# jwheo12/RustRayTrace

Measured on AMD Instinct MI355X. Metric: Mrays/sec + wall-clock for 1920×1080×512spp RTOW final scene, higher is better.
Workload: dtype f32; 1 GPU; C2 RTOW final scene (gpu/mod.rs generator, seed 0x5EED1234), 1920x1080x512spp, max_depth 100, 486 spheres; spp=512, max_depth=100, parallelism=whole frame on 1 GPU (the band split with one rank), no gather

## Files before the change

include/rrt_hip.h:

```cpp
#ifndef RRT_HIP_H
#define RRT_HIP_H

#include <stddef.h>
#include <stdint.h>

#ifdef __cplusplus
extern "C" {
#endif

#define RRT_ABI_VERSION 11u


typedef struct RrtCamera {
    float origin[4];
    float pixel00[4];
    float pixel_delta_u[4];
    float pixel_delta_v[4];
    float u[4];
    float v[4];
    float background[4];
    float params_f[4];
    uint32_t params_u[4];
} RrtCamera;

// ... 301 lines not shown
int32_t rrt_quantize_accum_books_async(uint32_t n_pixels, const float *d_accum, uint32_t samples_per_pixel,
                                       uint8_t *d_rgb8, void *stream);
int32_t rrt_quantize_accum_books_f64_async(uint32_t n_pixels, const double *d_accum, uint32_t samples_per_pixel,
                                           uint8_t *d_rgb8, void *stream);

int32_t rrt_hip_render_f64_rgb8(const RrtCamera *cam,
                                const RrtSphere *spheres, uint32_t n_spheres,
                                const RrtMaterial *materials, uint32_t n_materials,
                                const RrtTexture *textures, uint32_t n_textures,
                                uint32_t total_spp, uint32_t n_gpus, uint32_t flags,
                                uint8_t *rgb8_out);

int32_t rrt_format_pnm_from_rgb8(uint32_t width, uint32_t height, const uint8_t *rgb8, int32_t binary,
                                 char *buf, size_t cap, size_t *written);
int32_t rrt_write_pnm_from_rgb8(uint32_t width, uint32_t height, const uint8_t *rgb8, int32_t binary,
                                const char *path);

int32_t rrt_device_count(int32_t *count);

void rrt_testing_device_wrap(int32_t on);

void rrt_testing_f64_layout(int32_t layout);

typedef struct RrtLaunchPlanQuery {
    uint32_t n_nodes, n_prims, stack_depth, node_stride;
    uint32_t book, specular, image_tex, n_perlin;
    uint32_t n_media, n_quads, f64, bvh4_in_lds;
    uint32_t min_waves, global_waves, _pad[2];
} RrtLaunchPlanQuery;
typedef struct RrtLaunchPlan {
    uint32_t ok, f64;
    int32_t kernel_class, shape;
    uint32_t stack_bytes, threads, waves, waves_noise_free;
    uint32_t scene_in_lds, perlin_in_lds, inv_r_in_lds, rec32_in_lds;
    uint32_t raise_limit, _pad;
    uint64_t lds_bytes;
} RrtLaunchPlan;
int32_t rrt_testing_launch_plan(const RrtLaunchPlanQuery *query, RrtLaunchPlan *plan);

int32_t rrt_testing_recip_check(uint64_t *mismatches);

int32_t rrt_testing_trig32_check(double *out);

int32_t rrt_testing_sqrt64_check(uint64_t *out);

enum RrtDeviceOp {
// ... 37 lines not shown
```

rustraytrace_amd/_lib.py:

```python
from __future__ import annotations

import ctypes
import os
from ctypes import POINTER, c_char_p, c_double, c_float, c_int32, c_size_t, c_uint8, c_uint32, c_uint64, c_void_p

import numpy as np

PKG_DIR = os.path.dirname(os.path.abspath(__file__))
LIB_PATH = os.environ.get("RRT_LIB_PATH") or os.path.join(PKG_DIR, "librrt_hip.so")

CAMERA_DTYPE = np.dtype(
    [
        ("origin", "<f4", 4),
        ("pixel00", "<f4", 4),
        ("pixel_delta_u", "<f4", 4),
        ("pixel_delta_v", "<f4", 4),
        ("u", "<f4", 4),
        ("v", "<f4", 4),
        ("background", "<f4", 4),
        ("params_f", "<f4", 4),
        ("params_u", "<u4", 4),
    ]
)
SPHERE_DTYPE = np.dtype([("center_radius", "<f4", 4), ("material_index", "<u4"), ("_pad", "<u4", 3)])
# ... 31 lines not shown
    "rrt_hip_render_rgb8",
    "rrt_hip_render_rgb8_ex",
    "rrt_quantize_accum_books",
    "rrt_quantize_accum_async",
    "rrt_format_pnm_from_rgb8",
    "rrt_write_pnm_from_rgb8",
    "rrt_hip_render_ex",
    "rrt_scene_create_ex",
    "rrt_build_bvh_ex",
    "rrt_build_bvh_binned",
    "rrt_scene_read_bvh",
    "rrt_build_next_week_scene",
    "rrt_build_rest_of_your_life_scene",
    "rrt_flatten_scene",
    "rrt_device_count",
    "rrt_hip_render_f64",
    "rrt_render_tile_f64_async",
    "rrt_quantize_accum_books_f64",
    "rrt_quantize_accum_books_async",
    "rrt_quantize_accum_books_f64_async",
    "rrt_hip_render_f64_rgb8",
    "rrt_testing_device_wrap",
    "rrt_testing_f64_layout",
    "rrt_testing_launch_plan",
    "rrt_testing_recip_check",
    "rrt_testing_trig32_check",
    "rrt_testing_sqrt64_check",
    "rrt_testing_device_ops",
    "rrt_testing_div_check",
    "rrt_testing_device_ops64",
)

DEVICE_OPS = {
    "SIN": (0, 1, 1), "COS": (1, 1, 1), "LOG": (2, 1, 1), "ACOS": (3, 1, 1), "ATAN2": (4, 2, 1),
    "DIV_A": (5, 2, 4), "DIV_CONST": (6, 1, 4), "FLOOR_I32": (7, 1, 1), "CHECKER": (8, 4, 1),
    "PERLIN": (9, 3, 8), "VEC": (10, 9, 13), "QUAD": (11, 9, 2), "SPHERE": (12, 11, 13),
}

DEVICE_OPS64 = {
    "ACOS64": (0, 1, 1), "ATAN2_64": (1, 2, 1), "DIV_A64": (2, 2, 3), "DIV_CONST64": (3, 1, 4), "SQRT64": (4, 1, 1),
    "AS_I32": (5, 1, 1), "ATT64": (6, 2, 4), "VEC64": (7, 9, 11), "TEXEL64": (8, 5, 6), "SPHERE64": (9, 11, 6),
}


class RrtTexture(ctypes.Structure):
    _fields_ = [("rgb8", POINTER(c_uint8)), ("width", c_int32), ("height", c_int32)]
# ... 201 lines not shown
        "rrt_hip_render_rgb8_ex": (c_int32, [P, P, c_uint32, P, c_uint32, P, c_uint32, P, c_uint32, c_uint32, c_uint32,
                                             P]),
        "rrt_quantize_accum_async": (c_int32, [c_uint32, P, c_uint32, P, P]),
        "rrt_format_pnm_from_rgb8": (c_int32, [c_uint32, c_uint32, P, c_int32, P, c_size_t, P]),
        "rrt_write_pnm_from_rgb8": (c_int32, [c_uint32, c_uint32, P, c_int32, c_char_p]),
        "rrt_hip_render_ex": (c_int32, [P, P, c_uint32, P, c_uint32, P, c_uint32, P, c_uint32, c_uint32, c_uint32, P]),
        "rrt_scene_create_ex": (c_int32, [P, P, c_uint32, P, c_uint32, P, c_uint32, P, c_uint32, c_int32, P]),
        "rrt_build_bvh_ex": (c_int32, [P, c_uint32, P, c_uint32, c_uint32, P, c_size_t, P, P]),
        "rrt_build_bvh_binned": (c_int32, [P, c_uint32, P, c_uint32, c_double, c_uint32, P, c_size_t, P, P]),
        "rrt_scene_read_bvh": (c_int32, [P, P, c_size_t, P]),
        "rrt_build_next_week_scene": (c_int32, [c_int32, P, c_uint64, P]),
        "rrt_build_rest_of_your_life_scene": (c_int32, [P, c_uint64, P]),
        "rrt_flatten_scene": (c_int32, [P, c_uint32, P, c_uint32, c_uint32, P]),
        "rrt_device_count": (c_int32, [P]),
        "rrt_hip_render_f64": (c_int32, [P, P, c_uint32, P, c_uint32, P, c_uint32, c_uint32, c_uint32, c_uint32, P]),
        "rrt_render_tile_f64_async": (c_int32, [P, P, P, P]),
        "rrt_quantize_accum_books_f64": (c_int32, [c_uint32, c_uint32, P, c_uint32, P]),
        "rrt_quantize_accum_books_async": (c_int32, [c_uint32, P, c_uint32, P, P]),
        "rrt_quantize_accum_books_f64_async": (c_int32, [c_uint32, P, c_uint32, P, P]),
        "rrt_hip_render_f64_rgb8": (c_int32, [P, P, c_uint32, P, c_uint32, P, c_uint32, c_uint32, c_uint32, c_uint32,
                                              P]),
        "rrt_testing_device_wrap": (None, [c_int32]),
        "rrt_testing_f64_layout": (None, [c_int32]),
        "rrt_testing_launch_plan": (c_int32, [P, P]),
        "rrt_testing_recip_check": (c_int32, [P]),
        "rrt_testing_trig32_check": (c_int32, [P]),
        "rrt_testing_sqrt64_check": (c_int32, [P]),
        "rrt_testing_device_ops": (c_int32, [c_uint32, c_uint32, P, P, P]),
        "rrt_testing_device_ops64": (c_int32, [c_uint32, c_uint32, P, P, P]),
        "rrt_testing_div_check": (c_int32, [P, c_uint32, P]),
    }
    experiment = "RRT_LIB_PATH" in os.environ
    for name, (res, args) in sig.items():
        if experiment and not hasattr(lib, name):
            continue
        fn = getattr(lib, name)
        fn.restype = res
        fn.argtypes = args
    _LIB = lib
    return lib


def check(rc: int) -> None:
    if rc != 0:
        msg = load().rrt_hip_last_error()
        raise RrtError(rc, msg.decode() if msg else "")
# ... 27 lines not shown
```

rustraytrace_amd/csrc/rrt_books64.hip:

```cpp
#include "rrt_internal.h"
#include "../../include/rrt_hip.h"

#include <atomic>
#include <cstdlib>
#include <type_traits>

namespace rrt {
namespace {

#include "rrt_device.h"
#include "rrt_box32.h"
#include "rrt_sphere32.h"

constexpr int kPrioRefill = 2, kPrioNode = 1, kPrioLeaf = 2, kPrioShade = 0;

#ifndef RRT_F64_STATS
#define RRT_F64_STATS 0
#endif
#ifndef RRT_DEBUG_NOREJECT
#define RRT_DEBUG_NOREJECT 0
#endif
__device__ __forceinline__ uint32_t wave_max_u32(uint32_t v) {
#pragma unroll
    for (int off = 32; off > 0; off >>= 1) v = max(v, (uint32_t)__shfl_xor((int)v, off, 64));
// ... 393 lines not shown
    uint32_t rx, ry, rz;
};
__device__ __forceinline__ RayK64 ray_consts64(D3 o, D3 d) {
    RayK64 r;
    r.b = box32_ray(o.x, o.y, o.z, d.x, d.y, d.z);
    r.ox = r.b.ix < 0.0f ? 16u : 0u;
    r.oy = r.b.iy < 0.0f ? 48u : 32u;
    r.oz = r.b.iz < 0.0f ? 80u : 64u;
    r.rx = r.b.ix < 0.0f ? 16u : 0u;
    r.ry = r.b.iy < 0.0f ? 16u : 0u;
    r.rz = r.b.iz < 0.0f ? 16u : 0u;
    return r;
}

struct Trav64 {
    double closest;
    float closest32;
    int hit_prim;
    int node;
    int sp;
};

template <bool kCount, typename Node, typename Stack>
__device__ __forceinline__ bool trav_node64(const Node *__restrict__ nodes, Stack &stack, const RayK64 &rk,
                                            Trav64 &t, Leaves &lv, Counters &cnt) {
    if (kCount) { cnt.nodes++; cnt.boxes += 2; }
    bool h0, h1;
    uint32_t l0, l1;
    float tn0 = 0.0f, tn1 = 0.0f;
    if constexpr (std::is_same<Node, GNode>::value) {
        const char *bx = reinterpret_cast<const char *>(nodes) + __umul24((uint32_t)t.node, 112u);
        auto quad = [&](uint32_t byte_off) { return *reinterpret_cast<const float4 *>(bx + byte_off); };
        const float4 x = quad(rk.ox), y = quad(rk.oy), z = quad(rk.oz);
        h0 = box32_hit(x.x, x.y, y.x, y.y, z.x, z.y, rk.b, t.closest32, tn0);
        h1 = box32_hit(x.z, x.w, y.z, y.w, z.z, z.w, rk.b, t.closest32, tn1);
        const uint2 lk = *reinterpret_cast<const uint2 *>(bx + 96);
        l0 = lk.x;
        l1 = lk.y;
    } else {
        const uint4 *q = reinterpret_cast<const uint4 *>(nodes + t.node);
        const uint4 a = q[0], b = q[1];
        auto ord = [](uint32_t w, uint32_t r) { return __builtin_amdgcn_alignbit(w, w, r); };
        const uint32_t x0 = ord(a.x, rk.rx), y0 = ord(a.y, rk.ry), z0 = ord(a.z, rk.rz);
        const uint32_t x1 = ord(a.w, rk.rx), y1 = ord(b.x, rk.ry), z1 = ord(b.y, rk.rz);
        h0 = box32_hit(lo16(x0), hi16(x0), lo16(y0), hi16(y0), lo16(z0), hi16(z0), rk.b, t.closest32, tn0);
        h1 = box32_hit(lo16(x1), hi16(x1), lo16(y1), hi16(y1), lo16(z1), hi16(z1), rk.b, t.closest32, tn1);
        l0 = b.z;
        l1 = b.w;
    }
    const uint32_t c0 = h0 ? (l0 >> kLinkCountShift) : 0u;
    const uint32_t c1 = h1 ? (l1 >> kLinkCountShift) : 0u;
    lv = c0 ? l0 + (c1 << kLinkCountShift) : l1;
    if (c0) h0 = false;
    if (c1) h1 = false;
    if (h0 && h1) {
        const bool first1 = tn1 < tn0;
        stack.store(t.sp, first1 ? (int)l0 : (int)l1);
        ++t.sp;
        t.node = first1 ? (int)l1 : (int)l0;
    } else if (h0) {
        t.node = (int)l0;
    } else if (h1) {
        t.node = (int)l1;
    } else if (t.sp == 0) {
        t.node = -1;
    } else {
        --t.sp;
        t.node = stack.load(t.sp);
    }
    return (c0 | c1) != 0;
}

__device__ __forceinline__ double recip_a64(double a) {
    if (!(a >= 0x1.0p-64 && a <= 0x1.0p64)) return 0.0;
    double r = __builtin_amdgcn_rcp(a);
    double e = __builtin_fma(-a, r, 1.0);
    r = __builtin_fma(r, e, r);
    e = __builtin_fma(-a, r, 1.0);
    return __builtin_fma(r, e, r);
}
__device__ __forceinline__ double div_a64_short(double n, double a, double ra) {
    const double q = n * ra;
    return __builtin_fma(__builtin_fma(-a, q, n), ra, q);
}
__device__ __forceinline__ bool div_a64_in_band(double r) { return __builtin_fabs(r) >= 0x1.0p-896; }
__device__ __forceinline__ double div_a64(double n, double a, double ra) {
    const double r = div_a64_short(n, a, ra);
    return div_a64_in_band(r) ? r : n / a;
}
__device__ __forceinline__ double root64(double h, double sq, double a, double ra) {
    const double n1 = h - sq, n2 = h + sq;
    double root = div_a64_short(n1, a, ra);
    if (!(0.001 < root)) root = div_a64_short(n2, a, ra);
// ... 325 lines not shown
        const uint32_t min_active = (live * P.trav_frac) >> 8;
        const uint32_t leaf_min = (live * P.leaf_frac) >> 8;
        if constexpr (RRT_F64_STATS == 1) {
            const uint64_t t = __builtin_amdgcn_s_memtime();
            ph0 += t - tp;
            tp = t;
        }
        RayK64 rk;
        double a = 0.0;
        if (tr.node >= 0) {
            rk = ray_consts64(ps.o, ps.d);
            a = dot(ps.d, ps.d);
        }
        __builtin_amdgcn_s_setprio(kPrioNode);
        Leaves lv = 0;
        for (;;) {
            if constexpr (RRT_F64_STATS == 4) {
                const uint64_t sm = __ballot(tr.node >= 0 && lv == 0);
                if (sm != 0) {
                    ph0 += 1;
                    ph1 += (uint64_t)__popcll(sm);
                }
            }
            if (tr.node >= 0 && lv == 0) {
                Leaves l;
                if (trav_node64<kCount>(nodes, stack, rk, tr, l, cnt)) lv = l;
            }
            const uint64_t pm = __ballot(lv != 0);
            const uint64_t tm = __ballot(tr.node >= 0) | pm;
            const bool leave = (uint32_t)__popcll(tm) <= min_active;
            const bool batch = ((uint32_t)__popcll(pm) > leaf_min) | leave | (tm == pm);
            if ((pm != 0) & batch) {
                __builtin_amdgcn_s_setprio(kPrioLeaf);
                [[maybe_unused]] const uint32_t n_l = lv >> kLinkCountShift, s_l = cnt.d1;
                if (lv != 0) {
                    leaves64<kCount>(prims, recs32, lv, ps.o, ps.d, a, P.sphere32 != 0u, tr, cnt);
                    lv = 0;
                }
                if constexpr (RRT_F64_STATS == 2) {
                    ph0 += wave_max_u32(n_l);
                    ph1 += wave_max_u32(cnt.d1 - s_l);
                    ph2 += 1;
                }
                if constexpr (RRT_F64_STATS == 4) ph2 += 64;
                __builtin_amdgcn_s_setprio(kPrioNode);
            }
            if (leave) break;
        }
        if constexpr (RRT_F64_STATS == 1) {
            const uint64_t t = __builtin_amdgcn_s_memtime();
// ... 561 lines not shown
```

rustraytrace_amd/csrc/rrt_device.h:

```cpp
#pragma once

__device__ __forceinline__ uint32_t wave_slot() {
    return (uint32_t)__builtin_amdgcn_readfirstlane(threadIdx.x) == threadIdx.x ? 64u : 0u;
}

__device__ __forceinline__ float lo16(uint32_t v) { return (float)__builtin_bit_cast(_Float16, (uint16_t)(v & 0xffffu)); }
__device__ __forceinline__ float hi16(uint32_t v) { return (float)__builtin_bit_cast(_Float16, (uint16_t)(v >> 16)); }

__device__ __forceinline__ uint64_t splitmix64(uint64_t z) {
    z += 0x9e3779b97f4a7c15ull;
    z = (z ^ (z >> 30)) * 0xbf58476d1ce4e5b9ull;
    z = (z ^ (z >> 27)) * 0x94d049bb133111ebull;
    return z ^ (z >> 31);
}
struct RngState {
    uint32_t a, b, c, d;
};
__device__ __forceinline__ uint32_t rotl32(uint32_t x, int k) { return (x << k) | (x >> (32 - k)); }
__device__ __forceinline__ uint32_t xor3_32(uint32_t x, uint32_t y, uint32_t z) {
#if defined(__gfx950__)
    return __builtin_amdgcn_bitop3_b32(x, y, z, 0x96);
#else
    return x ^ y ^ z;
#endif
// ... 17 lines not shown
    s.c ^= s.a;
    s.d ^= s.b;
    s.b ^= s.c;
    s.a ^= s.d;
    s.c ^= t;
    s.d = rotl32(s.d, 11);
    return r;
}
__device__ __forceinline__ RngState rng_seed(uint64_t z, uint64_t key) {
    return RngState{(uint32_t)z, (uint32_t)(z >> 32), (uint32_t)key, (uint32_t)(key >> 32) | 1u};
}
__device__ __forceinline__ uint64_t rng_key(const RngState &s) { return (uint64_t)s.a | ((uint64_t)s.b << 32); }
__device__ __forceinline__ float rnd(RngState &s) { return (float)(rng_next(s) >> 8) * 0x1.0p-24f; }
__device__ __forceinline__ float rnd_range(RngState &s, float lo, float hi) { return rnd(s) * (hi - lo) + lo; }
__device__ __forceinline__ float rnd_pm1(RngState &s) {
    return __builtin_fmaf((float)(rng_next(s) >> 8), 0x1.0p-23f, -1.0f);
}

struct Counters {
    uint32_t nodes, boxes, spheres;
    uint32_t d0, d1, d2;
};

template <typename StackT, int kBlk>
struct LdsStack {
    StackT *base;
    __device__ __forceinline__ void init(StackT *lds, uint32_t tid) {
        if constexpr (sizeof(StackT) == 2) {
            const uint32_t lane = tid & 63u;
            base = lds + (tid & ~63u) + ((lane & 31u) << 1) + (lane >> 5);
        } else {
            base = lds + tid;
        }
    }
    __device__ __forceinline__ void store(int sp, int v) { base[sp * kBlk] = (StackT)v; }
    __device__ __forceinline__ int load(int sp) const { return (int)base[sp * kBlk]; }
};

using Leaves = uint32_t;

__device__ __forceinline__ const __attribute__((address_space(4))) KParams *kernarg_params() {
    auto q = (const __attribute__((address_space(4))) KParams *)__builtin_amdgcn_kernarg_segment_ptr();
    asm volatile("" : "+s"(q));
    return q;
}
template <class FD>
__device__ __forceinline__ FastDiv fdiv(const FD &f) { return FastDiv{f.m, f.s}; }

template <class KP>
__device__ __forceinline__ uint64_t pixel_key(const KP &P, uint32_t x, uint32_t y) {
    return splitmix64(((uint64_t)P.seed << 32) ^ (uint64_t)(y * P.width + x));
}
__device__ __forceinline__ RngState path_rng_k(uint64_t key, uint32_t s) { return rng_seed(splitmix64(key + s), key); }

template <class KP>
__host__ __device__ __forceinline__ uint32_t chunk_first(const KP &P, uint32_t c) {
    return c < P.n_big ? c * P.chunk : P.n_big * P.chunk + (c - P.n_big) * P.chunk_small;
}

// ... 6 lines not shown
```

rustraytrace_amd/csrc/rrt_host.cpp:

```cpp
#include "rrt_internal.h"
#include "rrt_bvh_binned.h"
#include "../../include/rrt_hip.h"

#include <algorithm>
#include <limits>
#include <atomic>
#include <chrono>
#include <cmath>
#include <cstdio>
#include <cstdlib>
#include <cstring>
#include <functional>
#include <mutex>
#include <string>
#include <thread>
#include <vector>

namespace {

thread_local std::string g_err;

int fail(int code, const std::string &msg) {
    g_err = msg;
    return code;
// ... 1838 lines not shown
    const size_t elem = scene->f64 ? sizeof(rrt::D4) : sizeof(float4);
    HIP_TRY(hipMalloc((void **)&scratch, std::max<size_t>((size_t)p.tile_rows * p.width, 1) * elem),
            "hipMalloc scratch accum");
    p.accum = scratch;
    p.accum64 = reinterpret_cast<rrt::D4 *>(scratch);
    p.counters = scene->d_work_counters;
    hipError_t e = hipMemset(scene->d_work_counters, 0, 8 * sizeof(unsigned long long));
    if (e == hipSuccess) e = rrt::launch_render_counting(p, nullptr);
    if (e == hipSuccess) e = hipDeviceSynchronize();
    unsigned long long c[8] = {0};
    if (e == hipSuccess) e = hipMemcpy(c, scene->d_work_counters, sizeof(c), hipMemcpyDeviceToHost);
    (void)hipFree(scratch);
    if (e != hipSuccess) return fail(RRT_E_HIP, std::string("counting render failed: ") + hipGetErrorString(e));
    *out = RrtCounters{c[0], c[1], c[2], c[3], c[4]};
    return RRT_OK;
}

}

static std::atomic<bool> g_device_wrap{false};
extern "C" void rrt_testing_device_wrap(int32_t on) { g_device_wrap.store(on != 0); }

extern "C" void rrt_testing_f64_layout(int32_t layout) { rrt::set_f64_layout(layout); }

extern "C" int32_t rrt_testing_launch_plan(const RrtLaunchPlanQuery *q, RrtLaunchPlan *out) {
    if (!q || !out) return fail(RRT_E_INVALID, "null query or out");
    *out = RrtLaunchPlan{};
    if (q->node_stride != 32u && q->node_stride != 80u && q->node_stride != 128u)
        return fail(RRT_E_INVALID, "node_stride must be 80 (staged BVH2), 32 (global BVH2) or 128 (BVH4)");
    if (q->book > 3u || q->book == 1u) return fail(RRT_E_INVALID, "book must be 0 (book 1), 2 or 3");
    rrt::KParams p{};
    static float4 some_motion;
    p.n_nodes = q->n_nodes;
    p.n_prims = q->n_prims;
    p.stack_depth = q->stack_depth;
    p.bvh_width = q->node_stride == 128u ? 4u : 2u;
    p.scene_in_lds = q->node_stride == 128u ? q->bvh4_in_lds : q->node_stride == 80u ? 1u : 0u;
    p.prim_motion = q->book ? &some_motion : nullptr;
    p.flags = (q->book == 3u ? RRT_FLAG_BOOK3 | RRT_FLAG_RAY_TIME : 0u) | (q->f64 ? RRT_FLAG_F64 : 0u);
    p.specular = q->specular;
    p.image_tex = q->image_tex;
    p.n_perlin = q->n_perlin;
    p.n_media = q->n_media;
    p.n_quads = q->n_quads;
    p.sphere32 = q->f64 ? 1u : 0u;
    p.min_waves = q->min_waves ? q->min_waves : 6u;
// ... 1200 lines not shown
```

rustraytrace_amd/csrc/rrt_internal.h:

```cpp
#pragma once

#include <hip/hip_runtime.h>
#include <stdint.h>

namespace rrt {

struct alignas(16) GNode {
    float box[2][9];
    uint32_t link[2];
};
static_assert(sizeof(GNode) == 80, "GNode must be 80 B");
struct alignas(16) GNodeH {
    uint32_t c0[3];
    uint32_t c1[3];
    uint32_t link[2];
};
static_assert(sizeof(GNodeH) == 32, "GNodeH must be 32 B");
constexpr uint32_t kLinkCountShift = 28;
constexpr uint32_t kLinkFirstMask = (1u << kLinkCountShift) - 1u;
constexpr uint32_t kMaxLeafPrims = 7;
constexpr uint32_t kMaxUnbounded = 4;

struct alignas(16) GNode4 {
    float4 lox, hix, loy, hiy, loz, hiz;
    int4 child;
    int4 count;
};
static_assert(sizeof(GNode4) == 128, "GNode4 must be 128 B");

struct alignas(16) GMaterial {
    float4 a;
    int4 b;
};

struct alignas(16) GPerlin {
    float4 randvec[256];
    uint32_t perm[256];
};

struct alignas(16) GQuad {
    float4 q;
    float4 u;
    float4 v;
// ... 246 lines not shown
```

rustraytrace_amd/csrc/rrt_kernel.hip:

```cpp
#include "rrt_internal.h"
#include "../../include/rrt_hip.h"

#include <algorithm>
#include <cstdio>
#include <cstdlib>
#include <type_traits>

namespace rrt {
namespace {

#ifndef RRT_PHASE_TIMING
#define RRT_PHASE_TIMING 0
#endif
#ifndef RRT_DEBUG_NOREJECT
#define RRT_DEBUG_NOREJECT 0
#endif
#ifndef RRT_DEBUG_EXTRA_NODE_LOAD
#define RRT_DEBUG_EXTRA_NODE_LOAD 0
#endif
#ifndef RRT_PRIO_REFILL
#define RRT_PRIO_REFILL 2
#endif
#ifndef RRT_PRIO_NODE
#define RRT_PRIO_NODE 1
#endif
#ifndef RRT_PRIO_LEAF
// ... 118 lines not shown
    if (x == 0.0f) {
        if (y > 0.0f) return kPiO2;
        if (y < 0.0f) return -kPiO2;
        return 0.0f;
    }
    float z = rrt_atanf(y / x);
    if (x < 0.0f) z = (y < 0.0f) ? z - kPi : z + kPi;
    return z;
}

__device__ __forceinline__ bool box_hit(float lx, float hx, float ly, float hy, float lz, float hz,
                                        V3 inv, V3 oi, float tmin, float tmax, float &tnear) {
    const float x0 = __builtin_fmaf(lx, inv.x, -oi.x), x1 = __builtin_fmaf(hx, inv.x, -oi.x);
    const float y0 = __builtin_fmaf(ly, inv.y, -oi.y), y1 = __builtin_fmaf(hy, inv.y, -oi.y);
    const float z0 = __builtin_fmaf(lz, inv.z, -oi.z), z1 = __builtin_fmaf(hz, inv.z, -oi.z);
    const float nr = __builtin_fmaxf(__builtin_fmaxf(__builtin_fminf(x0, x1), __builtin_fminf(y0, y1)),
                                     __builtin_fmaxf(__builtin_fminf(z0, z1), tmin));
    const float fr = __builtin_fminf(__builtin_fminf(__builtin_fmaxf(x0, x1), __builtin_fmaxf(y0, y1)),
                                     __builtin_fminf(__builtin_fmaxf(z0, z1), tmax));
    tnear = nr;
    return nr < fr;
}

__device__ __forceinline__ bool box_hit_ordered(float nx, float fx, float ny, float fy, float nz, float fz, V3 inv,
                                                V3 oi, float tmin, float tmax, float &tnear) {
    const float x0 = __builtin_fmaf(nx, inv.x, -oi.x), x1 = __builtin_fmaf(fx, inv.x, -oi.x);
    const float y0 = __builtin_fmaf(ny, inv.y, -oi.y), y1 = __builtin_fmaf(fy, inv.y, -oi.y);
    const float z0 = __builtin_fmaf(nz, inv.z, -oi.z), z1 = __builtin_fmaf(fz, inv.z, -oi.z);
    const float nr = __builtin_fmaxf(__builtin_fmaxf(x0, y0), __builtin_fmaxf(z0, tmin));
    const float fr = __builtin_fminf(__builtin_fminf(x1, y1), __builtin_fminf(z1, tmax));
    tnear = nr;
    return nr < fr;
}


struct RayK {
    V3 inv;
    V3 oi;
    float a;
    float ra;
    uint32_t ox, oy, oz;
};

__device__ __forceinline__ float clamp_inv(float v) { return __builtin_fmaxf(__builtin_fminf(v, 0x1.0p64f), -0x1.0p64f); }
__device__ __forceinline__ float clamped_slope(float s) {
    return __builtin_fabsf(s) < 0x1.0p-126f ? __builtin_copysignf(0x1.0p64f, s) : clamp_inv(recip_rn(s));
}

#ifndef RRT_F16_ORDERED_MAX_CLASS
#define RRT_F16_ORDERED_MAX_CLASS 3
#endif
#ifndef RRT_B1U_WAVES
#define RRT_B1U_WAVES 8
// ... 255 lines not shown
            cr = prim_cr.at(i);
        }
        const V3 oc = v3(cr.x - o.x, cr.y - o.y, cr.z - o.z);
        const float h = dot(d, oc);
        const float c = dot(oc, oc) - (PR::kR2 ? cr.w : cr.w * cr.w);
        const float disc = __builtin_fmaf(h, h, -(a * c));
        if (disc < 0.0f) continue;
        if constexpr (RRT_PHASE_TIMING == 3) cnt.d2 += 1;
        const float sq = sqrt_rn(disc);
        float root = div_by_a(h - sq, rk);
        if (!(0.001f < root)) root = div_by_a(h + sq, rk);
        if (0.001f < root && root < closest) {
            closest = root;
            hit_prim = i;
        }
    }
}


struct Trav {
    float closest;
    int hit_prim;
    int node;
    int sp;
};

__device__ __forceinline__ void trav_begin(Trav &t) {
    t.closest = __builtin_inff();
    t.hit_prim = -1;
    t.node = 0;
    t.sp = 0;
}


template <bool kCount, bool kOrd16, typename Node, typename Stack>
__device__ __forceinline__ bool trav_node(const Node *__restrict__ nodes, Stack &stack, const RayK &rk, Trav &t,
                                          Leaves &lv, Counters &cnt) {
    if (kCount) { cnt.nodes++; cnt.boxes += 2; }
    float tn0 = 0.0f, tn1 = 0.0f;
    bool h0, h1;
    uint32_t l0, l1;
    if constexpr (std::is_same<Node, GNode>::value) {
        const GNode &n = *reinterpret_cast<const GNode *>(reinterpret_cast<const char *>(nodes) +
                                                           __umul24((uint32_t)t.node, (uint32_t)sizeof(GNode)));
        const char *bx = reinterpret_cast<const char *>(&n.box[0][0]);
        auto plane = [&](uint32_t byte_off) { return *reinterpret_cast<const float *>(bx + byte_off); };
        h0 = box_hit_ordered(plane(rk.ox), plane(rk.ox + 4), plane(rk.oy), plane(rk.oy + 4), plane(rk.oz),
                             plane(rk.oz + 4), rk.inv, rk.oi, 0.001f, t.closest, tn0);
        h1 = box_hit_ordered(plane(rk.ox + 36), plane(rk.ox + 40), plane(rk.oy + 36), plane(rk.oy + 40),
                             plane(rk.oz + 36), plane(rk.oz + 40), rk.inv, rk.oi, 0.001f, t.closest, tn1);
        l0 = n.link[0];
        l1 = n.link[1];
    } else {
        const uint4 *q = reinterpret_cast<const uint4 *>(nodes + t.node);
        const uint4 a = q[0], b = q[1];
#if RRT_DEBUG_EXTRA_NODE_LOAD == 1
        {
            const uint4 *q2 = q;
            asm volatile("" : "+v"(q2));
            const uint4 c = q2[0];
            asm volatile("" ::"v"(c.x ^ c.y ^ c.z ^ c.w));
        }
#endif
#if RRT_DEBUG_EXTRA_NODE_LOAD == 2
        uint32_t dep_zero;
        {
            uint32_t z = a.x;
            asm volatile("v_and_b32 %0, 0, %0" : "+v"(z));
            const uint4 c = q[z];
            dep_zero = c.x;
            asm volatile("v_and_b32 %0, 0, %0" : "+v"(dep_zero));
        }
#endif
        if (kOrd16) {
            auto ord = [](uint32_t w, uint32_t r) { return __builtin_amdgcn_alignbit(w, w, r); };
            uint32_t ry, rz;
            asm volatile("v_lshrrev_b32 %0, 5, %1" : "=v"(ry) : "v"(rk.ox));
            asm volatile("v_lshrrev_b32 %0, 10, %1" : "=v"(rz) : "v"(rk.ox));
            const uint32_t x0 = ord(a.x, rk.ox), y0 = ord(a.y, ry), z0 = ord(a.z, rz);
            const uint32_t x1 = ord(a.w, rk.ox), y1 = ord(b.x, ry), z1 = ord(b.y, rz);
            h0 = box_hit_ordered(lo16(x0), hi16(x0), lo16(y0), hi16(y0), lo16(z0), hi16(z0), rk.inv, rk.oi, 0.001f,
                                 t.closest, tn0);
            h1 = box_hit_ordered(lo16(x1), hi16(x1), lo16(y1), hi16(y1), lo16(z1), hi16(z1), rk.inv, rk.oi, 0.001f,
                                 t.closest, tn1);
        } else {
            h0 = box_hit(lo16(a.x), hi16(a.x), lo16(a.y), hi16(a.y), lo16(a.z), hi16(a.z), rk.inv, rk.oi, 0.001f, t.closest, tn0);
            h1 = box_hit(lo16(a.w), hi16(a.w), lo16(b.x), hi16(b.x), lo16(b.y), hi16(b.y), rk.inv, rk.oi, 0.001f, t.closest, tn1);
        }
        l0 = b.z;
        l1 = b.w;
#if RRT_DEBUG_EXTRA_NODE_LOAD == 2
        l0 += dep_zero;
        l1 += dep_zero;
#endif
    }
    const uint32_t c0 = h0 ? (l0 >> kLinkCountShift) : 0u;
    const uint32_t c1 = h1 ? (l1 >> kLinkCountShift) : 0u;
    lv = c0 ? l0 + (c1 << kLinkCountShift) : l1;
    if (c0) h0 = false;
    if (c1) h1 = false;
    if (h0 && h1) {
        const bool first1 = tn1 < tn0;
        stack.store(t.sp, first1 ? (int)l0 : (int)l1);
        ++t.sp;
        t.node = first1 ? (int)l1 : (int)l0;
    } else if (h0) {
        t.node = (int)l0;
    } else if (h1) {
        t.node = (int)l1;
    } else if (t.sp == 0) {
        t.node = -1;
    } else {
        --t.sp;
        t.node = stack.load(t.sp);
    }
    return (c0 | c1) != 0;
}

template <bool kCount, bool kHoldRa, class PR>
__device__ __forceinline__ void trav_leaves(const PR &prims, Leaves lv, V3 o, V3 d, const RayK &rk_, int skip, Trav &t,
                                            Counters &cnt) {
    RayK rk = rk_;
    if (!kHoldRa) rk.ra = refine_ra(rk.a);
    const int first = (int)(lv & kLinkFirstMask), count = (int)(lv >> kLinkCountShift);
    test_range<kCount>(prims, first, count, o, d, rk, skip, t.closest, t.hit_prim, cnt);
}

template <bool kCount, typename Stack, class PR>
__device__ __forceinline__ bool trav_step4(const GNode4 *__restrict__ nodes, const PR &prims,
                                           Stack &stack, V3 o, V3 d, const RayK &rk, int skip, Trav &t, Counters &cnt) {
    const GNode4 n = nodes[t.node];
    if (kCount) { cnt.nodes++; cnt.boxes += 4; }
    const float lox[4] = {n.lox.x, n.lox.y, n.lox.z, n.lox.w}, hix[4] = {n.hix.x, n.hix.y, n.hix.z, n.hix.w};
    const float loy[4] = {n.loy.x, n.loy.y, n.loy.z, n.loy.w}, hiy[4] = {n.hiy.x, n.hiy.y, n.hiy.z, n.hiy.w};
    const float loz[4] = {n.loz.x, n.loz.y, n.loz.z, n.loz.w}, hiz[4] = {n.hiz.x, n.hiz.y, n.hiz.z, n.hiz.w};
    const int child[4] = {n.child.x, n.child.y, n.child.z, n.child.w};
    const int count[4] = {n.count.x, n.count.y, n.count.z, n.count.w};
    float key[4];
    int idx[4];
// ... 561 lines not shown
    ps.k++;
    ps.skip = exit_skip(is_quad, is_medium, front, dir, nrm, prim);
    return false;
}

template <int kBook2, bool kNoise, typename C, class PR>
__device__ __forceinline__ bool shade_any(const KParams &P, const PR &prims, const GMaterial *mtl, PathState &ps,
                                          float t, int prim, V3 &sum, C &cnt) {
    if constexpr (kBook2 == 4) return shade_b3<kNoise>(P, prims, mtl, ps, t, prim, sum, cnt);
    else return shade<kBook2, kNoise>(P, prims, mtl, ps, t, prim, sum, cnt);
}

__device__ __forceinline__ void trace_segment(uint32_t xy, uint32_t s, const PathState &ps, float t, int prim) {
#ifdef RRT_TRACE_X
    if ((xy & 0xffffu) == RRT_TRACE_X && (xy >> 16) == RRT_TRACE_Y && s == RRT_TRACE_S)
        printf("K k=%u o=(%a %a %a) d=(%a %a %a) t=%a prim=%d T=(%a %a %a) rng=%llx\n", ps.k, ps.o.x, ps.o.y, ps.o.z,
               ps.d.x, ps.d.y, ps.d.z, t, prim, ps.T.x, ps.T.y, ps.T.z, (unsigned long long)rng_key(ps.rng));
#endif
}

template <bool kLds, bool kCount, typename StackT, bool kWide, int kBook2, int kBlk, bool kNoise>
__device__ __forceinline__ void render_body(const KParams &P) {
    extern __shared__ uint4 lds_dyn[];
    StackT *lds_stack = reinterpret_cast<StackT *>(lds_dyn);
    using Node = typename std::conditional<kWide, GNode4, typename std::conditional<kLds, GNode, GNodeH>::type>::type;
    const Node *nodes = reinterpret_cast<const Node *>(P.nodes);
    const float4 *prims = P.prim_cr;
    const GMaterial *mtl = P.prim_mtl;
    const float4 *motion = P.prim_motion;
    if constexpr (kLds) {
        uint4 *dst = lds_dyn + (P.stack_depth * kBlk * sizeof(StackT) + 15u) / 16u;
        const uint4 *src_n = reinterpret_cast<const uint4 *>(P.nodes);
        const uint32_t nn = P.n_nodes * (uint32_t)(sizeof(Node) / 16);
        for (uint32_t i = threadIdx.x; i < nn; i += kBlk) dst[i] = src_n[i];
        const uint4 *src_p = reinterpret_cast<const uint4 *>(P.prim_cr);
        for (uint32_t i = threadIdx.x; i < P.n_prims; i += kBlk) dst[nn + i] = src_p[i];
        const uint4 *src_m = reinterpret_cast<const uint4 *>(P.prim_mtl);
        const uint32_t nm = P.n_prims * (uint32_t)(sizeof(GMaterial) / 16);
        for (uint32_t i = threadIdx.x; i < nm; i += kBlk) dst[nn + P.n_prims + i] = src_m[i];
        if constexpr (kBook2 > 0) {
            const uint4 *src_v = reinterpret_cast<const uint4 *>(P.prim_motion);
            for (uint32_t i = threadIdx.x; i < P.n_prims; i += kBlk) dst[nn + P.n_prims + nm + i] = src_v[i];
        }
        __syncthreads();
        nodes = reinterpret_cast<const Node *>(dst);
        prims = reinterpret_cast<const float4 *>(dst + nn);
        mtl = reinterpret_cast<const GMaterial *>(dst + nn + P.n_prims);
        if constexpr (kBook2 > 0) motion = reinterpret_cast<const float4 *>(dst + nn + P.n_prims + nm);
    }
    const GPerlin *perlin = P.perlin;
    if constexpr (kBook2 > 0) {
        if (P.perlin_in_lds) {
            size_t off16 = (P.stack_depth * kBlk * sizeof(StackT) + 15u) / 16u;
            if constexpr (kLds) off16 += P.n_nodes * (uint32_t)(sizeof(Node) / 16) + 3u * P.n_prims + P.n_prims;
            uint4 *dst = lds_dyn + off16;
            const uint4 *src = reinterpret_cast<const uint4 *>(P.perlin);
            const uint32_t n16 = P.n_perlin * (uint32_t)(sizeof(GPerlin) / 16);
            for (uint32_t i = threadIdx.x; i < n16; i += kBlk) dst[i] = src[i];
            __syncthreads();
            perlin = reinterpret_cast<const GPerlin *>(dst);
        }
    }
    LdsStack<StackT, kBlk> stack;
    stack.init(lds_stack, threadIdx.x);

    const uint32_t lane = threadIdx.x & 63u;
    Counters cnt = {0, 0, 0, 0, 0, 0};
    uint32_t w_rays = 0, w_paths = 0;
    uint32_t has = 0;
    bool q_open = true;
    uint32_t xy = 0, s = 0, s_hi = 0;
    uint64_t pkey = 0;
    V3 sum = v3(0.0f, 0.0f, 0.0f);
    PathState ps;
    Trav tr;
    tr.node = -1;
    uint32_t need_ray = 0;
    uint32_t pool_base = (blockIdx.x & (kQueues - 1u)) * 64u, pool_left = 0;
    [[maybe_unused]] uint64_t ph0 = 0, ph1 = 0, ph2 = 0, tp = 0;
    for (;;) {
        if constexpr (RRT_PHASE_TIMING == 1) tp = __builtin_amdgcn_s_memtime();
        if constexpr (RRT_PHASE_TIMING == 2) ph2++;
        __builtin_amdgcn_s_setprio(RRT_PRIO_REFILL);
        uint64_t idle = __ballot(!has);
        if (idle != 0 && pool_left == 0 && q_open) {
// ... 36 lines not shown
                        xy = x | (y << 16);
                        s = Q.sample_begin + chunk_first(Q, chunk);
                        s_hi = min(s + (chunk < Q.n_big ? Q.chunk : Q.chunk_small), Q.sample_end);
                        sum = v3(0.0f, 0.0f, 0.0f);
                        pkey = pixel_key(Q, x, y);
                        ps.rng = path_rng_k(pkey, s);
                        camera_ray<kBook2 == 4>(P, x, y, s, ps, cnt);
                        need_ray = 1;
                        has = 1;
                    }
                }
            }
            pool_base += n;
            pool_left -= n;
        }
        if (__ballot(has) == 0) break;

        uint32_t seg_done = 0;
        uint32_t started = 0;
        if (has && need_ray) {
            if (ps.k >= P.max_depth) {
                seg_done = 1;
            } else {
                trav_begin(tr);
                need_ray = 0;
                started = 1;
            }
        }
        w_rays += (uint32_t)__popcll(__ballot(started));
        const uint32_t live = (uint32_t)__popcll(__ballot(has));
        const uint32_t min_active = (live * P.trav_frac) >> 8;
        if constexpr (RRT_PHASE_TIMING == 1) {
            const uint64_t t = __builtin_amdgcn_s_memtime();
            ph0 += t - tp;
            tp = t;
        }
        RayK rk;
        constexpr bool kOrd16 = !kLds && !kWide && kBook2 <= RRT_F16_ORDERED_MAX_CLASS;
        constexpr bool kHoldRa = !(kOrd16 && kBook2 == 3);
        if (tr.node >= 0) rk = ray_consts<!kOrd16, kHoldRa>(ps.o, ps.d);
        const Prims<kBook2> pr{prims, motion, ps.time, P.quads, P.media, P.n_quads, rng_key(ps.rng) ^ ((uint64_t)ps.k << 32), perlin};
        if constexpr (kWide) {
            for (;;) {
                if constexpr (RRT_PHASE_TIMING == 2) {
                    ph0 += 64;
                    ph1 += (uint64_t)__popcll(__ballot(tr.node >= 0));
                }
                if (tr.node >= 0) trav_step4<kCount>(nodes, pr, stack, ps.o, ps.d, rk, ps.skip, tr, cnt);
                if ((uint32_t)__popcll(__ballot(tr.node >= 0)) <= min_active) break;
            }
        } else {
            const uint32_t leaf_min = (live * P.leaf_frac) >> 8;
            __builtin_amdgcn_s_setprio(RRT_PRIO_NODE);
            Leaves lv = 0;
            for (;;) {
                if constexpr (RRT_PHASE_TIMING == 2) {
                    ph0 += 64;
                    ph1 += (uint64_t)__popcll(__ballot(tr.node >= 0 && lv == 0));
                }
                if constexpr (RRT_PHASE_TIMING == 8) {
                    const bool stepping = tr.node >= 0 && lv == 0;
                    const uint64_t sm = __ballot(stepping);
                    const int n0 = __builtin_amdgcn_readfirstlane(stepping ? tr.node : 0x7fffffff);
                    const uint64_t same = __ballot(stepping && tr.node == n0);
                    if (sm != 0) {
                        ph0 += 64;
                        if (same == sm) {
                            ph1 += 64;
                            ph2 += (uint64_t)__popcll(sm);
                        }
                    }
                }
                if (tr.node >= 0 && lv == 0) {
                    Leaves l;
                    if (trav_node<kCount, kOrd16>(nodes, stack, rk, tr, l, cnt)) lv = l;
                }
                const uint64_t pm = __ballot(lv != 0);
                const uint64_t tm = __ballot(tr.node >= 0) | pm;
                const bool leave = (uint32_t)__popcll(tm) <= min_active;
                const bool batch = ((uint32_t)__popcll(pm) > leaf_min) | leave | (tm == pm);
                if ((pm != 0) & batch) {
                    __builtin_amdgcn_s_setprio(RRT_PRIO_LEAF);
                    if (lv != 0) {
                        trav_leaves<kCount, kHoldRa>(pr, lv, ps.o, ps.d, rk, ps.skip, tr, cnt);
                        lv = 0;
                    }
                    __builtin_amdgcn_s_setprio(RRT_PRIO_NODE);
                }
                if (leave) break;
            }
        }
        __builtin_amdgcn_s_setprio(RRT_PRIO_SHADE);
        if constexpr (RRT_PHASE_TIMING == 1) {
            const uint64_t t = __builtin_amdgcn_s_memtime();
            ph1 += t - tp;
            tp = t;
        }
        const bool shading = has && !need_ray && tr.node < 0;
        if (shading) {
            need_ray = 1;
            const Prims<kBook2> spr{prims, motion, ps.time, P.quads, P.media, P.n_quads, rng_key(ps.rng) ^ ((uint64_t)ps.k << 32), perlin};
            if constexpr (Prims<kBook2>::kHasMedia) {
                if (!kHoldRa) rk.ra = refine_ra(rk.a);
                for (uint32_t u = P.n_prims - P.n_unbounded; u < P.n_prims; ++u) {
                    if (kCount) cnt.spheres++;
                    const int m = (int)(-prims[u].w) - 1 - (int)P.n_quads;
                    float tm;
                    if (medium_hit(spr, m, ps.o, ps.d, rk, tr.closest, tm)) {
                        tr.closest = tm;
// ... 223 lines not shown
    pl.raise_limit = best > kLdsDefaultMax ? 1u : 0u;
    return pl;
}

bool perlin_fits_lds(KParams p) {
    if (p.n_perlin == 0 || !p.prim_motion) return false;
    p.perlin_in_lds = 1u;
    const LaunchPlan pl = plan_launch(p);
    return pl.ok && !pl.raise_limit;
}

namespace {

template <bool kLds, typename StackT, bool kWide, int kBook2, int kArm>
hipError_t launch_variant(const KParams &p, const LaunchPlan &pl, bool count, hipStream_t stream) {
    constexpr ArmShape kS = arm_shape(kBook2, kArm, kLds);
    constexpr int kWaves = kS.waves, kWavesNF = kS.waves_nf, kBlk = kS.threads;
    static_assert(kS.stack_bytes == (int)sizeof(StackT), "stack type of the launch shape");
    constexpr bool kNoiseFree = kBook2 > 0 && sizeof(StackT) == 2;
    if (p.n_units == 0) return hipSuccess;
    if (pl.arm != kArm || pl.kclass != kBook2 || pl.threads != (uint32_t)kBlk || pl.scene_in_lds != (kLds ? 1u : 0u) ||
        (p.bvh_width == 4) != kWide)
        return hipErrorInvalidValue;
    const size_t lds = (size_t)pl.lds_bytes;
    auto kernel = count                       ? rrt_render<kLds, true, StackT, kWide, kWaves, kBook2, kBlk, (kBook2 > 0)>
                  : !kNoiseFree || p.n_perlin ? rrt_render<kLds, false, StackT, kWide, kWaves, kBook2, kBlk, (kBook2 > 0)>
                                              : rrt_render<kLds, false, StackT, kWide, kWavesNF, kBook2, kBlk, false>;
    hipError_t e;
    if (pl.raise_limit) {
        e = hipFuncSetAttribute(reinterpret_cast<const void *>(kernel), hipFuncAttributeMaxDynamicSharedMemorySize,
                                (int)lds);
        if (e != hipSuccess) return e;
    }
    int per_cu = 0;
    e = hipOccupancyMaxActiveBlocksPerMultiprocessor(&per_cu, kernel, kBlk, lds);
    if (e != hipSuccess) return e;
    if (per_cu < 1) per_cu = 1;
    const uint32_t want = (p.n_units + kBlk - 1) / kBlk;
    const uint32_t blocks = std::max<uint32_t>(std::min<uint32_t>(want, (uint32_t)per_cu * p.n_cus), kQueues);
    e = hipMemsetAsync(p.unit_counter, 0, kQueues * 32u * sizeof(uint32_t), stream);
    if (e != hipSuccess) return e;
    hipLaunchKernelGGL(kernel, dim3(blocks), dim3(kBlk), lds, stream, p);
    e = hipGetLastError();
    static const bool log = std::getenv("RRT_LAUNCH_LOG") != nullptr;
    if (log)
        std::fprintf(stderr, "rrt launch: class %d, %d x %d, stack %d B x %u, %zu B of LDS%s, %d block(s)/CU, %u blocks: %s\n",
// ... 290 lines not shown
```

Measured before the change: 34140 Mrays/s.

## Store BVH links as LDS byte addresses and use pointer-based LDS stack

When the binary BVH is copied into LDS, child links are rewritten into absolute LDS byte addresses, so node fetches skip the index multiply. The traversal stack moves to the end of the LDS block and becomes a byte-address pointer with push and top helpers. The leaf-link decode is simplified, and the traversal loop uses precomputed ballot masks with inverse_ballot to pick active lanes. The slab test also uses a raw v_min_f32 for the final clamp. The LDS layout changes, and a new guard rejects scenes whose node bytes exceed what 16-bit stack entries can address.

```diff
diff --git a/include/rrt_hip.h b/include/rrt_hip.h
--- a/include/rrt_hip.h
+++ b/include/rrt_hip.h
@@ -347,6 +347,8 @@
 
 void rrt_testing_f64_layout(int32_t layout);
 
+uint32_t rrt_testing_lds_node_link(uint32_t link);
+
 typedef struct RrtLaunchPlanQuery {
     uint32_t n_nodes, n_prims, stack_depth, node_stride;
     uint32_t book, specular, image_tex, n_perlin;
diff --git a/rustraytrace_amd/_lib.py b/rustraytrace_amd/_lib.py
--- a/rustraytrace_amd/_lib.py
+++ b/rustraytrace_amd/_lib.py
@@ -77,6 +77,7 @@
     "rrt_hip_render_f64_rgb8",
     "rrt_testing_device_wrap",
     "rrt_testing_f64_layout",
+    "rrt_testing_lds_node_link",
     "rrt_testing_launch_plan",
     "rrt_testing_recip_check",
     "rrt_testing_trig32_check",
@@ -324,6 +325,7 @@
                                               P]),
         "rrt_testing_device_wrap": (None, [c_int32]),
         "rrt_testing_f64_layout": (None, [c_int32]),
+        "rrt_testing_lds_node_link": (c_uint32, [c_uint32]),
         "rrt_testing_launch_plan": (c_int32, [P, P]),
         "rrt_testing_recip_check": (c_int32, [P]),
         "rrt_testing_trig32_check": (c_int32, [P]),
diff --git a/rustraytrace_amd/csrc/rrt_books64.hip b/rustraytrace_amd/csrc/rrt_books64.hip
--- a/rustraytrace_amd/csrc/rrt_books64.hip
+++ b/rustraytrace_amd/csrc/rrt_books64.hip
@@ -439,7 +439,7 @@
 };
 
 template <bool kCount, typename Node, typename Stack>
-__device__ __forceinline__ bool trav_node64(const Node *__restrict__ nodes, Stack &stack, const RayK64 &rk,
+__device__ __forceinline__ void trav_node64(const Node *__restrict__ nodes, Stack &stack, const RayK64 &rk,
                                             Trav64 &t, Leaves &lv, Counters &cnt) {
     if (kCount) { cnt.nodes++; cnt.boxes += 2; }
     bool h0, h1;
@@ -465,11 +465,11 @@
         l0 = b.z;
         l1 = b.w;
     }
-    const uint32_t c0 = h0 ? (l0 >> kLinkCountShift) : 0u;
-    const uint32_t c1 = h1 ? (l1 >> kLinkCountShift) : 0u;
-    lv = c0 ? l0 + (c1 << kLinkCountShift) : l1;
-    if (c0) h0 = false;
-    if (c1) h1 = false;
+    const bool f0 = h0 && l0 > kLinkFirstMask, f1 = h1 && l1 > kLinkFirstMask;
+    const uint32_t m1 = f1 ? l1 : 0u;
+    lv = f0 ? l0 + (m1 & ~kLinkFirstMask) : m1;
+    if (f0) h0 = false;
+    if (f1) h1 = false;
     if (h0 && h1) {
         const bool first1 = tn1 < tn0;
         stack.store(t.sp, first1 ? (int)l0 : (int)l1);
@@ -485,7 +485,6 @@
         --t.sp;
         t.node = stack.load(t.sp);
     }
-    return (c0 | c1) != 0;
 }
 
 __device__ __forceinline__ double recip_a64(double a) {
@@ -857,10 +856,7 @@
                     ph1 += (uint64_t)__popcll(sm);
                 }
             }
-            if (tr.node >= 0 && lv == 0) {
-                Leaves l;
-                if (trav_node64<kCount>(nodes, stack, rk, tr, l, cnt)) lv = l;
-            }
+            if (tr.node >= 0 && lv == 0) trav_node64<kCount>(nodes, stack, rk, tr, lv, cnt);
             const uint64_t pm = __ballot(lv != 0);
             const uint64_t tm = __ballot(tr.node >= 0) | pm;
             const bool leave = (uint32_t)__popcll(tm) <= min_active;
diff --git a/rustraytrace_amd/csrc/rrt_device.h b/rustraytrace_amd/csrc/rrt_device.h
--- a/rustraytrace_amd/csrc/rrt_device.h
+++ b/rustraytrace_amd/csrc/rrt_device.h
@@ -63,9 +63,14 @@
     uint32_t d0, d1, d2;
 };
 
+template <class T>
+using LdsPtr = __attribute__((address_space(3))) T *;
+__device__ __forceinline__ uint32_t lds_addr(const void *p) { return (uint32_t)(uintptr_t)(LdsPtr<const char>)p; }
 template <typename StackT, int kBlk>
 struct LdsStack {
+    static constexpr uint32_t kStride = (uint32_t)kBlk * (uint32_t)sizeof(StackT);
     StackT *base;
+    uint32_t bottom;
     __device__ __forceinline__ void init(StackT *lds, uint32_t tid) {
         if constexpr (sizeof(StackT) == 2) {
             const uint32_t lane = tid & 63u;
@@ -73,9 +78,15 @@
         } else {
             base = lds + tid;
         }
+        bottom = lds_addr(base);
     }
     __device__ __forceinline__ void store(int sp, int v) { base[sp * kBlk] = (StackT)v; }
     __device__ __forceinline__ int load(int sp) const { return (int)base[sp * kBlk]; }
+    static __device__ __forceinline__ void push(uint32_t &sp, int v) {
+        *(LdsPtr<StackT>)(uintptr_t)sp = (StackT)v;
+        sp += kStride;
+    }
+    static __device__ __forceinline__ int top(uint32_t sp) { return (int)*(LdsPtr<const StackT>)(uintptr_t)sp; }
 };
 
 using Leaves = uint32_t;
diff --git a/rustraytrace_amd/csrc/rrt_host.cpp b/rustraytrace_amd/csrc/rrt_host.cpp
--- a/rustraytrace_amd/csrc/rrt_host.cpp
+++ b/rustraytrace_amd/csrc/rrt_host.cpp
@@ -1884,6 +1884,8 @@
 extern "C" void rrt_testing_device_wrap(int32_t on) { g_device_wrap.store(on != 0); }
 
 extern "C" void rrt_testing_f64_layout(int32_t layout) { rrt::set_f64_layout(layout); }
+
+extern "C" uint32_t rrt_testing_lds_node_link(uint32_t link) { return rrt::lds_node_link(link); }
 
 extern "C" int32_t rrt_testing_launch_plan(const RrtLaunchPlanQuery *q, RrtLaunchPlan *out) {
     if (!q || !out) return fail(RRT_E_INVALID, "null query or out");
diff --git a/rustraytrace_amd/csrc/rrt_internal.h b/rustraytrace_amd/csrc/rrt_internal.h
--- a/rustraytrace_amd/csrc/rrt_internal.h
+++ b/rustraytrace_amd/csrc/rrt_internal.h
@@ -19,6 +19,9 @@
 constexpr uint32_t kLinkCountShift = 28;
 constexpr uint32_t kLinkFirstMask = (1u << kLinkCountShift) - 1u;
 constexpr uint32_t kMaxLeafPrims = 7;
+__host__ __device__ constexpr uint32_t lds_node_link(uint32_t link) {
+    return link > kLinkFirstMask ? link : link * (uint32_t)sizeof(GNode);
+}
 constexpr uint32_t kMaxUnbounded = 4;
 
 struct alignas(16) GNode4 {
diff --git a/rustraytrace_amd/csrc/rrt_kernel.hip b/rustraytrace_amd/csrc/rrt_kernel.hip
--- a/rustraytrace_amd/csrc/rrt_kernel.hip
+++ b/rustraytrace_amd/csrc/rrt_kernel.hip
@@ -2,6 +2,7 @@
 #include "../../include/rrt_hip.h"
 
 #include <algorithm>
+#include <cstddef>
 #include <cstdio>
 #include <cstdlib>
 #include <type_traits>
@@ -166,13 +167,18 @@
     return nr < fr;
 }
 
+__device__ __forceinline__ float min_f32_raw(float a, float b) {
+    float r;
+    asm("v_min_f32 %0, %1, %2" : "=v"(r) : "v"(a), "v"(b));
+    return r;
+}
 __device__ __forceinline__ bool box_hit_ordered(float nx, float fx, float ny, float fy, float nz, float fz, V3 inv,
                                                 V3 oi, float tmin, float tmax, float &tnear) {
     const float x0 = __builtin_fmaf(nx, inv.x, -oi.x), x1 = __builtin_fmaf(fx, inv.x, -oi.x);
     const float y0 = __builtin_fmaf(ny, inv.y, -oi.y), y1 = __builtin_fmaf(fy, inv.y, -oi.y);
     const float z0 = __builtin_fmaf(nz, inv.z, -oi.z), z1 = __builtin_fmaf(fz, inv.z, -oi.z);
     const float nr = __builtin_fmaxf(__builtin_fmaxf(x0, y0), __builtin_fmaxf(z0, tmin));
-    const float fr = __builtin_fminf(__builtin_fminf(x1, y1), __builtin_fminf(z1, tmax));
+    const float fr = min_f32_raw(__builtin_fminf(__builtin_fminf(x1, y1), z1), tmax);
     tnear = nr;
     return nr < fr;
 }
@@ -474,35 +480,35 @@
     float closest;
     int hit_prim;
     int node;
-    int sp;
+    uint32_t sp;
 };
 
-__device__ __forceinline__ void trav_begin(Trav &t) {
+__device__ __forceinline__ void trav_begin(Trav &t, int root, uint32_t sp0) {
     t.closest = __builtin_inff();
     t.hit_prim = -1;
-    t.node = 0;
-    t.sp = 0;
+    t.node = root;
+    t.sp = sp0;
 }
 
 
 template <bool kCount, bool kOrd16, typename Node, typename Stack>
-__device__ __forceinline__ bool trav_node(const Node *__restrict__ nodes, Stack &stack, const RayK &rk, Trav &t,
+__device__ __forceinline__ void trav_node(const Node *__restrict__ nodes, Stack &stack, const RayK &rk, Trav &t,
                                           Leaves &lv, Counters &cnt) {
     if (kCount) { cnt.nodes++; cnt.boxes += 2; }
     float tn0 = 0.0f, tn1 = 0.0f;
     bool h0, h1;
     uint32_t l0, l1;
     if constexpr (std::is_same<Node, GNode>::value) {
-        const GNode &n = *reinterpret_cast<const GNode *>(reinterpret_cast<const char *>(nodes) +
-                                                           __umul24((uint32_t)t.node, (uint32_t)sizeof(GNode)));
-        const char *bx = reinterpret_cast<const char *>(&n.box[0][0]);
-        auto plane = [&](uint32_t byte_off) { return *reinterpret_cast<const float *>(bx + byte_off); };
+        static_assert(offsetof(GNode, box) == 0, "GNode planes start the record");
+        const uint32_t bx = (uint32_t)t.node;
+        auto plane = [&](uint32_t byte_off) { return *(LdsPtr<const float>)(uintptr_t)(bx + byte_off); };
         h0 = box_hit_ordered(plane(rk.ox), plane(rk.ox + 4), plane(rk.oy), plane(rk.oy + 4), plane(rk.oz),
                              plane(rk.oz + 4), rk.inv, rk.oi, 0.001f, t.closest, tn0);
         h1 = box_hit_ordered(plane(rk.ox + 36), plane(rk.ox + 40), plane(rk.oy + 36), plane(rk.oy + 40),
                              plane(rk.oz + 36), plane(rk.oz + 40), rk.inv, rk.oi, 0.001f, t.closest, tn1);
-        l0 = n.link[0];
-        l1 = n.link[1];
+        const LdsPtr<const uint32_t> lk = (LdsPtr<const uint32_t>)(uintptr_t)(bx + (uint32_t)offsetof(GNode, link));
+        l0 = lk[0];
+        l1 = lk[1];
     } else {
         const uint4 *q = reinterpret_cast<const uint4 *>(nodes + t.node);
         const uint4 a = q[0], b = q[1];
@@ -546,27 +552,25 @@
         l1 += dep_zero;
 #endif
     }
-    const uint32_t c0 = h0 ? (l0 >> kLinkCountShift) : 0u;
-    const uint32_t c1 = h1 ? (l1 >> kLinkCountShift) : 0u;
-    lv = c0 ? l0 + (c1 << kLinkCountShift) : l1;
-    if (c0) h0 = false;
-    if (c1) h1 = false;
+    const bool f0 = h0 && l0 > kLinkFirstMask, f1 = h1 && l1 > kLinkFirstMask;
+    const uint32_t m1 = f1 ? l1 : 0u;
+    lv = f0 ? l0 + (m1 & ~kLinkFirstMask) : m1;
+    if (f0) h0 = false;
+    if (f1) h1 = false;
     if (h0 && h1) {
         const bool first1 = tn1 < tn0;
-        stack.store(t.sp, first1 ? (int)l0 : (int)l1);
-        ++t.sp;
+        Stack::push(t.sp, first1 ? (int)l0 : (int)l1);
         t.node = first1 ? (int)l1 : (int)l0;
     } else if (h0) {
         t.node = (int)l0;
     } else if (h1) {
         t.node = (int)l1;
-    } else if (t.sp == 0) {
+    } else {
+        const bool more = t.sp != stack.bottom;
         t.node = -1;
-    } else {
-        --t.sp;
-        t.node = stack.load(t.sp);
-    }
-    return (c0 | c1) != 0;
+        t.sp -= Stack::kStride;
+        if (more) t.node = Stack::top(t.sp);
+    }
 }
 
 template <bool kCount, bool kHoldRa, class PR>
@@ -1174,25 +1178,39 @@
 template <bool kLds, bool kCount, typename StackT, bool kWide, int kBook2, int kBlk, bool kNoise>
 __device__ __forceinline__ void render_body(const KParams &P) {
     extern __shared__ uint4 lds_dyn[];
-    StackT *lds_stack = reinterpret_cast<StackT *>(lds_dyn);
+    uint32_t stack16 = 0;
+    [[maybe_unused]] const uint32_t node_base = kLds && !kWide ? lds_addr(lds_dyn) : 0u;
     using Node = typename std::conditional<kWide, GNode4, typename std::conditional<kLds, GNode, GNodeH>::type>::type;
     const Node *nodes = reinterpret_cast<const Node *>(P.nodes);
     const float4 *prims = P.prim_cr;
     const GMaterial *mtl = P.prim_mtl;
     const float4 *motion = P.prim_motion;
     if constexpr (kLds) {
-        uint4 *dst = lds_dyn + (P.stack_depth * kBlk * sizeof(StackT) + 15u) / 16u;
+        uint4 *dst = lds_dyn;
         const uint4 *src_n = reinterpret_cast<const uint4 *>(P.nodes);
-        const uint32_t nn = P.n_nodes * (uint32_t)(sizeof(Node) / 16);
-        for (uint32_t i = threadIdx.x; i < nn; i += kBlk) dst[i] = src_n[i];
+        constexpr uint32_t kNode16 = (uint32_t)(sizeof(Node) / 16);
+        const uint32_t nn = P.n_nodes * kNode16;
+        for (uint32_t i = threadIdx.x; i < nn; i += kBlk) {
+            uint4 v = src_n[i];
+            if constexpr (!kWide) {
+                static_assert(offsetof(GNode, link) == sizeof(GNode) - 8, "GNode links end the record");
+                if (i % kNode16 == kNode16 - 1u) {
+                    v.z = lds_node_link(v.z) + (v.z > kLinkFirstMask ? 0u : node_base);
+                    v.w = lds_node_link(v.w) + (v.w > kLinkFirstMask ? 0u : node_base);
+                }
+            }
+            dst[i] = v;
+        }
         const uint4 *src_p = reinterpret_cast<const uint4 *>(P.prim_cr);
         for (uint32_t i = threadIdx.x; i < P.n_prims; i += kBlk) dst[nn + i] = src_p[i];
         const uint4 *src_m = reinterpret_cast<const uint4 *>(P.prim_mtl);
         const uint32_t nm = P.n_prims * (uint32_t)(sizeof(GMaterial) / 16);
         for (uint32_t i = threadIdx.x; i < nm; i += kBlk) dst[nn + P.n_prims + i] = src_m[i];
+        stack16 = nn + P.n_prims + nm;
         if constexpr (kBook2 > 0) {
             const uint4 *src_v = reinterpret_cast<const uint4 *>(P.prim_motion);
             for (uint32_t i = threadIdx.x; i < P.n_prims; i += kBlk) dst[nn + P.n_prims + nm + i] = src_v[i];
+            stack16 += P.n_prims;
         }
         __syncthreads();
         nodes = reinterpret_cast<const Node *>(dst);
@@ -1203,16 +1221,18 @@
     const GPerlin *perlin = P.perlin;
     if constexpr (kBook2 > 0) {
         if (P.perlin_in_lds) {
-            size_t off16 = (P.stack_depth * kBlk * sizeof(StackT) + 15u) / 16u;
-            if constexpr (kLds) off16 += P.n_nodes * (uint32_t)(sizeof(Node) / 16) + 3u * P.n_prims + P.n_prims;
+            size_t off16 = stack16;
+            if constexpr (!kLds) off16 = (P.stack_depth * kBlk * sizeof(StackT) + 15u) / 16u;
             uint4 *dst = lds_dyn + off16;
             const uint4 *src = reinterpret_cast<const uint4 *>(P.perlin);
             const uint32_t n16 = P.n_perlin * (uint32_t)(sizeof(GPerlin) / 16);
             for (uint32_t i = threadIdx.x; i < n16; i += kBlk) dst[i] = src[i];
             __syncthreads();
             perlin = reinterpret_cast<const GPerlin *>(dst);
-        }
-    }
+            if constexpr (kLds) stack16 += n16;
+        }
+    }
+    StackT *lds_stack = reinterpret_cast<StackT *>(lds_dyn + stack16);
     LdsStack<StackT, kBlk> stack;
     stack.init(lds_stack, threadIdx.x);
 
@@ -1295,7 +1315,7 @@
             if (ps.k >= P.max_depth) {
                 seg_done = 1;
             } else {
-                trav_begin(tr);
+                trav_begin(tr, kWide ? 0 : (int)node_base, kWide ? 0u : stack.bottom);
                 need_ray = 0;
                 started = 1;
             }
@@ -1326,6 +1346,7 @@
             const uint32_t leaf_min = (live * P.leaf_frac) >> 8;
             __builtin_amdgcn_s_setprio(RRT_PRIO_NODE);
             Leaves lv = 0;
+            uint64_t step = __ballot(tr.node >= 0);
             for (;;) {
                 if constexpr (RRT_PHASE_TIMING == 2) {
                     ph0 += 64;
@@ -1344,20 +1365,20 @@
                         }
                     }
                 }
-                if (tr.node >= 0 && lv == 0) {
-                    Leaves l;
-                    if (trav_node<kCount, kOrd16>(nodes, stack, rk, tr, l, cnt)) lv = l;
-                }
+                if (__builtin_amdgcn_inverse_ballot_w64(step)) trav_node<kCount, kOrd16>(nodes, stack, rk, tr, lv, cnt);
                 const uint64_t pm = __ballot(lv != 0);
-                const uint64_t tm = __ballot(tr.node >= 0) | pm;
+                const uint64_t nm = __ballot(tr.node >= 0);
+                const uint64_t tm = nm | pm;
                 const bool leave = (uint32_t)__popcll(tm) <= min_active;
                 const bool batch = ((uint32_t)__popcll(pm) > leaf_min) | leave | (tm == pm);
+                step = nm & ~pm;
                 if ((pm != 0) & batch) {
                     __builtin_amdgcn_s_setprio(RRT_PRIO_LEAF);
-                    if (lv != 0) {
+                    if (__builtin_amdgcn_inverse_ballot_w64(pm)) {
                         trav_leaves<kCount, kHoldRa>(pr, lv, ps.o, ps.d, rk, ps.skip, tr, cnt);
                         lv = 0;
                     }
+                    step = nm;
                     __builtin_amdgcn_s_setprio(RRT_PRIO_NODE);
                 }
                 if (leave) break;
@@ -1627,6 +1648,7 @@
     if (pl.arm != kArm || pl.kclass != kBook2 || pl.threads != (uint32_t)kBlk || pl.scene_in_lds != (kLds ? 1u : 0u) ||
         (p.bvh_width == 4) != kWide)
         return hipErrorInvalidValue;
+    if (kLds && !kWide && sizeof(StackT) == 2 && (size_t)p.n_nodes * sizeof(GNode) > 65536u) return hipErrorInvalidValue;
     const size_t lds = (size_t)pl.lds_bytes;
     auto kernel = count                       ? rrt_render<kLds, true, StackT, kWide, kWaves, kBook2, kBlk, (kBook2 > 0)>
                   : !kNoiseFree || p.n_perlin ? rrt_render<kLds, false, StackT, kWide, kWaves, kBook2, kBlk, (kBook2 > 0)>
```

Result: faster. 35970 Mrays/s, median of 6 (+5.4%).
